# Coda-Research-Group/LearnedMetricIndex

Measured on AMD Instinct MI355X. Metric: queries/sec @ recall@10, 768-d 10M index, 10k query batch, higher is better.
Workload: dtype f16 prefilter (f32 accumulate) + f32 exact re-rank; outputs identical to the all-f32 path

## Files before the change

learnedmetricindex_amd/csrc/lmi_host_scan.h:

```cpp
#pragma once
#include "lmi_host.h"

static bool rescore_is_streamed(const lmi_index* h) {
    return h->rescore_streamed && rc_waves_for(h->dp, 4) > 0 && rc_wave_lds(h->dp, 4, true) <= RC_SMALL_LDS_CAP;
}
static int rescore_group_size(int nb) { return nb % 4 == 0 ? 4 : nb % 3 == 0 ? 3 : nb % 2 == 0 ? 2 : 1; }

struct ScanPlan {
    int nq, nb, kout, L;
    long long nslots;
    long long ncb_bound;
    long long ncols;
    int max_nch;
    long long part_lists;
    bool fast;
    bool low_d;
    bool ps_wide;
    int tile_cb;
    int sample_max;
    bool qbound;
    int primary_nb;
    bool use_front;
    bool streamed;
    int G, groups, sub_cap;
// ... 470 lines not shown
    F2.x.cap = 0;
    F2.x.fail = fbw + 2;
    F2.x.launch = 1;
    F2.head = F.head + 16;
    F2.redo_count = rc; F2.redo_bucket = rb; F2.redo_col = rcol;
    CHK(launch_pass2<false>(h, C.P, F2));
    return 0;
}

static void rescore_params(lmi_index* h, const ScanCall& C, const PrefilterParams& F, bool overflow_sorted, RescoreParams& Q) {
    const ScanPlan& P = C.P;
    unsigned* fbw = h->fb_list.as<unsigned>();
    Q.bucket_order = C.order;
    Q.slot_col = h->slot_col.as<int>();
    Q.nslots = (int)P.nslots;
    Q.nb = P.nb;
    Q.d = h->d;
    Q.raw = C.raw;
    Q.rb_start = h->d_rb_start.as<int>();
    Q.nb_rows = C.R.nb_rows;
    Q.cand_cnt = F.cand_cnt;
    Q.cand_row = F.cand_row;
    Q.cand_s = F.cand_s;
    Q.eps2 = F.eps2;
    Q.rows = h->rowmajor.as<float>();
    Q.dp = h->dp;
    Q.q = C.q;
    Q.qn2 = C.qn2;
    Q.ids_slab = h->ids_slab.as<unsigned>();
    Q.rank_d = h->rank_d.as<float>();
    Q.rank_id = h->rank_id.as<unsigned>();
    Q.fallback = h->fallback.as<int>();
    Q.nkeep = h->nkeep.as<int>();
    Q.fb_count = reinterpret_cast<int*>(fbw);
    Q.fb_list = reinterpret_cast<int*>(fbw + 8);
    Q.x_fail = fbw + 1;
    Q.x_off = overflow_sorted ? h->x_off.as<unsigned>() : nullptr;
    Q.x_ext = h->x_ext.as<uint2>();
    Q.x_log = F.x.log;
    Q.x_head = F.x.head;
    Q.x_cap = F.x.cap;
    Q.redo_col = overflow_sorted ? reinterpret_cast<const unsigned char*>(h->redo.as<unsigned>() + 1 + P.L) : nullptr;
    Q.ts = h->ts_set;
    Q.p2_end = p2_end_cell(h);
    if (Q.ts) { (void)tsp(h, ST_TAIL); (void)tsp(h, ST_P2END); (void)tsp(h, ST_FB); }
    Q.merge_pending = nullptr; Q.m_kout = 0; Q.m_out_d = nullptr; Q.m_out_id = nullptr; Q.m_out_key = nullptr;
#ifndef LMI_ABL_NOEMIT
    if (P.tail_merges) {
        Q.merge_pending = h->rs_flag.as<int>(); Q.m_kout = P.kout; Q.m_out_d = C.out_d; Q.m_out_id = C.out_id; Q.m_out_key = C.out_key;
        if (Q.ts) (void)tsp(h, ST_END);
    }
#endif
    Q.host_oflag = P.use_tail ? h->h_oflag : nullptr;
}
static Frag16 frag16_of(const lmi_index* h) {
    Frag16 F;
    F.frag = h->slab16.as<uint4>(); F.scale = h->xscale.as<float>(); F.KG16 = h->KG16; F.f16x16 = frag16x16(h);
    return F;
}

static int rerank(lmi_index* h, const ScanCall& C, const RescoreParams& Q) {
    const ScanPlan& P = C.P;
    const int nslots = (int)P.nslots, G = P.G, groups = P.groups;
    const bool f16 = h->storage == LMI_STORAGE_F16;
    if (!P.streamed) {
        if (f16) select_rescore_kernel<true><<<cdiv(nslots, RS_WAVES), 64 * RS_WAVES, 0, h->stream>>>(Q, frag16_of(h));
        else select_rescore_kernel<false><<<cdiv(nslots, RS_WAVES), 64 * RS_WAVES, 0, h->stream>>>(Q);
        HIPCHK(hipGetLastError());
        return 0;
    }
    CHK(h->surv_row.reserve((size_t)nslots * RC_KEEP * 4));
    SelectOut O;
    O.surv_row = h->surv_row.as<unsigned>();
    O.G = G;
    O.grp_flag = P.use_tail ? nullptr : h->rs_flag.as<int>();
    O.active = h->rs_active.as<int>();
    O.sub_cap = P.sub_cap;
    O.big = O.active + RC_SUB + RC_SUB * P.sub_cap;
    if (P.use_tail) {
        TailParams T;
        T.ngroups = groups; T.merge = P.tail_merges ? 1 : 0; T.kout = P.kout;
        T.out_d = C.out_d; T.out_id = C.out_id; T.out_key = C.out_key;
        T.pending = h->rs_flag.as<int>();
        const int lds_s = RC_WAVES * tail_wave_lds(h->dp, G, true);
        const int blocks = cdiv(groups, RC_WAVES);
#define LMI_TL_LAUNCH(GV) { if (f16) tail_kernel<GV, true><<<blocks, 64 * RC_WAVES, lds_s, h->stream>>>(Q, O, T, frag16_of(h)); \
                           else tail_kernel<GV><<<blocks, 64 * RC_WAVES, lds_s, h->stream>>>(Q, O, T); }
        if (G == 4) LMI_TL_LAUNCH(4) else if (G == 3) LMI_TL_LAUNCH(3) else if (G == 2) LMI_TL_LAUNCH(2) else LMI_TL_LAUNCH(1)
#undef LMI_TL_LAUNCH
        HIPCHK(hipGetLastError());
        return 0;
    }
    select_kernel<<<cdiv(nslots, 4), 256, 0, h->stream>>>(Q, O);
    HIPCHK(hipGetLastError());
    const int wb = rc_waves_for(h->dp, G), ws = rescore_small_waves(h->dp, G);
    h->last_plan[LMI_PLAN_RESCORE_SMALL_WAVES] = ws;
    const int blocks = cdiv(groups, ws);
    const int lds = wb * rc_wave_lds(h->dp, G), lds_s = ws * rc_wave_lds(h->dp, G, true);
#define LMI_RC_LAUNCH(GV) { if (f16) { rescore_kernel<GV, true, true><<<blocks, 64 * ws, lds_s, h->stream>>>(Q, O, frag16_of(h)); \
                                       rescore_kernel<GV, false, true><<<std::min(cdiv(groups, wb), h->num_cus), 64 * wb, lds, h->stream>>>(Q, O, frag16_of(h)); } \
                            else { rescore_kernel<GV, true><<<blocks, 64 * ws, lds_s, h->stream>>>(Q, O); \
                                   rescore_kernel<GV, false><<<std::min(cdiv(groups, wb), h->num_cus), 64 * wb, lds, h->stream>>>(Q, O); } }
    if (G == 4) LMI_RC_LAUNCH(4) else if (G == 3) LMI_RC_LAUNCH(3) else if (G == 2) LMI_RC_LAUNCH(2) else LMI_RC_LAUNCH(1)
#undef LMI_RC_LAUNCH
    HIPCHK(hipGetLastError());
    return 0;
}

static int scan_fallback(lmi_index* h, const ScanCall& C, const RescoreParams& Q) {
    if (h->storage == LMI_STORAGE_F16) fallback_kernel<true><<<std::min(cdiv(C.P.nslots, 4), h->num_cus * 4), 256, 0, h->stream>>>(Q, frag16_of(h));
    else fallback_kernel<false><<<std::min(cdiv(C.P.nslots, 4), h->num_cus * 4), 256, 0, h->stream>>>(Q);
    HIPCHK(hipGetLastError());
    return 0;
}

static int final_merge(lmi_index* h, const ScanCall& C) {
    const ScanPlan& P = C.P;
    const RouteArrays& R = C.R;
    MergeParams M;
    M.bucket_order = C.order;
    M.slot_col = h->slot_col.as<int>();
    M.nq = P.nq;
    M.nb = P.nb;
    M.L = P.L;
    M.kout = P.kout;
    M.raw = C.raw;
    M.skip_a = P.fast ? 1 : 0;
    M.rb_start = h->d_rb_start.as<int>();
    M.nb_rows = R.nb_rows;
    M.nch = R.nch;
    M.cb_start = R.cb_start;
    M.part_base = R.part_base;
    M.part_score = h->part_score.as<float>();
    M.part_row = h->part_row.as<unsigned>();
    M.ids_slab = h->ids_slab.as<unsigned>();
    M.qn2 = C.qn2;
    M.rank_d = h->rank_d.as<float>();
    M.rank_id = h->rank_id.as<unsigned>();
    M.ts = h->ts_set;
    M.scan_end = (!P.fast && h->ts_set) ? scan_end_cell(h) : nullptr;
    if (M.ts && !P.tail_merges) { (void)tsp(h, ST_MERGE); (void)tsp(h, ST_END); }
    M.out_d = C.out_d;
    M.out_id = C.out_id;
    M.out_key = C.out_key;
    const int kind = merge_kind(P);
    if (kind == 0) {  }
    else if (kind == 1) merge_ranks_kernel<<<cdiv(P.nq, 64), 64, 0, h->stream>>>(M);
    else merge_kernel<<<P.nq, 64, 0, h->stream>>>(M);
    HIPCHK(hipGetLastError());
    h->last_plan[LMI_PLAN_MERGE_KIND] = kind;
    return 0;
}

static int scan_enqueue(lmi_index* h, const float* d_qs, int nq, const int* d_order, int nb, int kout, int raw,
                        float* d_dists, uint32_t* d_ids, uint32_t* d_keys) {
    ScanCall C;
    C.P = scan_plan(h, nq, nb, kout);
    const ScanPlan& P = C.P;
    C.order = d_order; C.raw = raw;
    C.out_d = d_dists; C.out_id = d_ids; C.out_key = d_keys;
    plan_record(h, P, h->last_plan);
    CHK(scan_augment_l2(h, C, d_qs));
    CHK(scan_reserve(h, C));
    scan_route_arrays(h, P, C.R);
    CHK(P.use_front ? front_fused(h, C) : front_separate(h, C));
    if (!P.fast) {
        CHK(exact_scan(h, C));
    } else {
        CHK(record(h, 2));
        PrefilterParams F;
        prefilter_params(h, C, F);
        CHK(prefilter_passes(h, C, F));
        bool overflow_sorted = false;
        CHK(overflow_arm(h, P, &overflow_sorted));
        if (overflow_sorted) CHK(overflow_redo(h, C, F));
        h->last_plan[LMI_PLAN_OVERFLOW_SORTED] = overflow_sorted;
        RescoreParams Q;
        rescore_params(h, C, F, overflow_sorted, Q);
#ifndef LMI_ABL_NOEMIT
        CHK(rerank(h, C, Q));
#endif
// ... 42 lines not shown
```

learnedmetricindex_amd/csrc/lmi_rescore.h:

```cpp
#pragma once
#include <type_traits>

#include "lmi_prefilter.h"

namespace lmi {

#ifndef LMI_RC_ROWS
#define LMI_RC_ROWS 64
#endif
#ifndef LMI_RC_CHUNK
#define LMI_RC_CHUNK 32
#endif
#ifndef LMI_RC_DEPTH
#define LMI_RC_DEPTH 3
#endif
#ifndef LMI_RC_KEEP
#define LMI_RC_KEEP 256
#endif
constexpr int RC_ROWS = LMI_RC_ROWS;
constexpr int RC_CHUNK = LMI_RC_CHUNK;
constexpr int RC_DEPTH = LMI_RC_DEPTH;
constexpr int RC_KEEP = LMI_RC_KEEP;
constexpr int RC_PITCH = RC_CHUNK * 4 + 16;
constexpr int RC_PIECES = (RC_ROWS * RC_PITCH + 1023) / 1024;
// ... 39 lines not shown
                if (PERV <= 4 || i < nper) c += (int)__popcll(__ballot(key[i] >= probe));
            if (c >= KPB) T = probe;
        }
        pv = __uint_as_float(T ^ ((T >> 31) ? 0x80000000u : 0xffffffffu));
    }
    const float cut = pv - e2;
    const unsigned cbits = __float_as_uint(cut);
    const unsigned kcut = cut != cut ? 1u : cbits ^ ((cbits >> 31) ? 0xffffffffu : 0x80000000u);
    unsigned* out = O.surv_row + (size_t)p * RC_KEEP;
    unsigned nk = 0;
#pragma unroll
    for (int i = 0; i < PERV; ++i) {
        if (i < nper) {
            const bool keep = key[i] != 0u && key[i] >= kcut;
            const unsigned long long bal = __ballot(keep);
            if (keep) {
                const unsigned k = nk + (unsigned)__popcll(bal & ((1ull << lane) - 1ull));
                if (k < (unsigned)RC_KEEP) out[k] = row_base + (i < SPEC ? r_spec[i < SPEC ? i : 0] : cr[lane + 64 * i]);
            }
            nk += (unsigned)__popcll(bal);
        }
    }
    if (nk == 0u && lane < KPB) {
        const int b = bkt;
        const int rb0 = P.rb_start[b], n_b = P.nb_rows[b];
        P.rank_d[(size_t)p * KPB + lane] = P.raw ? -3.402823466e+38f : pad_dist(P.qn2);
        P.rank_id[(size_t)p * KPB + lane] = P.raw ? NOROW : P.ids_slab[(size_t)rb0 * 32 + (n_b - 1)];
    }
    if (lane == 0) {
        if (nk > (unsigned)RC_KEEP) flag_fallback(P, p);
        else {
            P.nkeep[p] = (int)nk;
            if (nk > 0 && atomicExch(&O.grp_flag[p / O.G], 1) == 0) {
                const int g = p / O.G, sub = g % RC_SUB;
                O.active[RC_SUB + sub * O.sub_cap + atomicAdd(&O.active[sub], 1)] = g;
            }
        }
    }
}

__global__ __launch_bounds__(256) void select_kernel(RescoreParams P, SelectOut O) {
    select_stamps(P);
    pf_x_scatter(P, blockIdx.x * 256 + threadIdx.x, gridDim.x * 256);
    const int wv = threadIdx.x >> 6, lane = threadIdx.x & 63;
    const int p = blockIdx.x * 4 + wv;
    if (p >= P.nslots) return;
    const float FMAXV = 3.402823466e+38f;
    const int col = P.slot_col[p];
    if (lane == 0) { P.fallback[p] = 0; P.nkeep[p] = 0; }
    if (col < 0) {
        if (lane < KPB) {
            P.rank_d[(size_t)p * KPB + lane] = P.raw ? -FMAXV : INFINITY;
            P.rank_id[(size_t)p * KPB + lane] = P.raw ? NOROW : 0u;
        }
        return;
    }
    const float* cs = P.cand_s + (size_t)col * PF_CAP;
    const unsigned* cr = P.cand_row + (size_t)col * PF_CAP;
    constexpr int PER = PF_CAP / 64;
    constexpr int SPEC = 4;
    float s_spec[SPEC];
    unsigned r_spec[SPEC];
#pragma unroll
    for (int i = 0; i < SPEC; ++i) { s_spec[i] = cs[lane + 64 * i]; r_spec[i] = cr[lane + 64 * i]; }
    const unsigned cnt = P.cand_cnt[col];
    if (cnt > (unsigned)PF_CAP) {
        if (lane == 0) flag_fallback(P, p);
        return;
    }
    if (cnt <= 64u) select_tail<1, SPEC>(P, O, p, col, lane, cnt, cs, cr, s_spec, r_spec);
    else if (cnt <= 256u) select_tail<4, SPEC>(P, O, p, col, lane, cnt, cs, cr, s_spec, r_spec);
    else select_tail<PER, SPEC>(P, O, p, col, lane, cnt, cs, cr, s_spec, r_spec);
}

constexpr int RC_SMALL_ROWS = 28;
#ifndef LMI_RC_SMALL_RING
#define LMI_RC_SMALL_RING (8 * 1024)
#endif
constexpr int RC_SMALL_LDS_CAP = 64 * 1024 + RC_WAVES * (LMI_RC_SMALL_RING - 8 * 1024);
constexpr int RC_SMALL_RING = LMI_RC_SMALL_RING;
__host__ __device__ inline int rc_wave_lds(int d, int G, bool small_form = false) {
    return small_form ? RC_SMALL_RING + d * 4 + 32 * 8 : RC_DEPTH * RC_BUF + d * 4 + G * RC_KEEP * 8;
}
__host__ inline int rc_waves_for(int d, int G) {
    for (int w = RC_WAVES; w >= 1; w >>= 1)
        if (w * rc_wave_lds(d, G) <= 160 * 1024 - 512) return w;
    return 0;
}
static_assert(RC_CHUNK % 32 == 0 && (RC_ROWS == 32 || RC_ROWS == 64) && RC_DEPTH >= 2 && RC_DEPTH <= 4, "rescore_kernel shapes");

template <int G, bool SMALL>
struct RcWave {
    static constexpr int RINGB = SMALL ? RC_SMALL_RING : RC_DEPTH * RC_BUF;
    static constexpr int KEEPW = SMALL ? 32 : G * RC_KEEP;
    unsigned char* mine;
    float* qs;
    unsigned* krow;
    float* ksc;
    __device__ __forceinline__ RcWave(unsigned char* base, int d) : mine(base), qs(reinterpret_cast<float*>(base + RINGB)),
        krow(reinterpret_cast<unsigned*>(base + RINGB + d * 4)), ksc(reinterpret_cast<float*>(base + RINGB + d * 4) + KEEPW) {}
    __device__ __forceinline__ void stage_query(const RescoreParams& P, int q, int lane) const {
        const int d = P.dp;
        const float* qg = P.q + (size_t)q * P.d;
        if (P.d == d) {
            for (int k = lane * 4; k < d; k += 256) *reinterpret_cast<float4*>(qs + k) = *reinterpret_cast<const float4*>(qg + k);
        } else {
            for (int k = lane; k < d; k += 64) qs[k] = k < P.d ? qg[k] : 0.0f;
        }
    }
};

template <int NP, int RINGB, bool H = false>
__device__ __forceinline__ void rc_run_batch(const RescoreParams& P, const Frag16& F, unsigned char* mine, const unsigned* krow, float* ksc, unsigned qaddr,
                                             int base, int total, int lane) {
    const int d = P.dp;
    const int n8 = (P.d + 7) >> 3;
    const int nchunks = H ? (n8 + 7) >> 3 : (d + RC_CHUNK - 1) / RC_CHUNK;
    float inv = 1.0f;
    if constexpr (H) inv = F.scale[1];
        constexpr int BUFB = NP * 1024;
        constexpr int DEPTH_RAW = RINGB / BUFB;
        constexpr int DEPTH = DEPTH_RAW > 16 ? 16 : ((DEPTH_RAW - 1) * NP > 60 ? 60 / NP + 1 : DEPTH_RAW);
        static_assert(DEPTH >= 2 && (DEPTH - 1) * NP <= 63, "vmcnt literal");
        const int nrows = min(RC_ROWS, total - base);
        const float* src[NP];
        unsigned colb[NP];
        int poff[H ? NP : 1];
#pragma unroll
        for (int pc = 0; pc < NP; ++pc) {
            const int o = pc * 1024 + lane * 16;
            const int r = o / RC_PITCH;
            const int cb = o - r * RC_PITCH;
            const bool okl = r < nrows && cb < RC_CHUNK * 4;
            const int i = base + (okl ? r : 0);
            if constexpr (H) {
                poff[pc] = okl ? 4 * frag16_piece_off(cb / 16, F.f16x16) : 0;
                src[pc] = reinterpret_cast<const float*>(F.frag + frag16_piece((long long)krow[i], 0, F.KG16, F.f16x16)) + poff[pc];
            } else {
                src[pc] = P.rows + (size_t)krow[i] * d + (okl ? cb / 4 : 0);
            }
            colb[pc] = okl ? (unsigned)cb : 0u;
        }
        auto issue = [&](int c, unsigned char* buf) {
            const int cbytes = H ? min(8, n8 - c * 8) * 16 : min(RC_CHUNK, d - c * RC_CHUNK) * 4;
#pragma unroll
            for (int pc = 0; pc < NP; ++pc) {
                const float* s_;
                if constexpr (H) s_ = src[pc] + c * 1024 - ((int)colb[pc] < cbytes ? 0 : poff[pc]);
                else s_ = src[pc] + c * RC_CHUNK - ((int)colb[pc] < cbytes ? 0 : (int)colb[pc] / 4);
                glds16(reinterpret_cast<const float4*>(s_), reinterpret_cast<float4*>(buf + pc * 1024));
            }
        };
        float acc = 0.0f;
#pragma unroll
        for (int c = 0; c < DEPTH - 1; ++c)
            if (c < nchunks) issue(c, mine + c * BUFB);
        int slot = 0;
        for (int c = 0; c < nchunks; ++c) {
            unsigned char* cur = mine + slot * BUFB;
            if (c + DEPTH - 1 < nchunks) {
                issue(c + DEPTH - 1, mine + (slot == 0 ? DEPTH - 1 : slot - 1) * BUFB);
                asm volatile("s_waitcnt vmcnt(%0)" :: "n"((DEPTH - 1) * NP) : "memory");
            } else {
                asm volatile("s_waitcnt vmcnt(0)" ::: "memory");
            }
            slot = slot + 1 == DEPTH ? 0 : slot + 1;
            if constexpr (H) {
              if (lane < nrows) {
                typedef float f32x4 __attribute__((ext_vector_type(4)));
                const unsigned xa = (unsigned)reinterpret_cast<uintptr_t>(cur) + (unsigned)lane * RC_PITCH;
                const unsigned qa = qaddr + (unsigned)c * 256u;
                const int np8 = min(8, n8 - c * 8);
                for (int st = 0; st * 4 < np8; ++st) {
                    f32x4 xv[4], qq[8];
                    const unsigned xo = xa + st * 64u, qo = qa + st * 128u;
                    asm volatile("ds_read_b128 %0, %12\n\tds_read_b128 %1, %12 offset:16\n\tds_read_b128 %2, %12 offset:32\n\t"
                                 "ds_read_b128 %3, %12 offset:48\n\t"
                                 "ds_read_b128 %4, %13\n\tds_read_b128 %5, %13 offset:16\n\tds_read_b128 %6, %13 offset:32\n\t"
                                 "ds_read_b128 %7, %13 offset:48\n\tds_read_b128 %8, %13 offset:64\n\tds_read_b128 %9, %13 offset:80\n\t"
                                 "ds_read_b128 %10, %13 offset:96\n\tds_read_b128 %11, %13 offset:112\n\ts_waitcnt lgkmcnt(0)"
                                 : "=&v"(xv[0]), "=&v"(xv[1]), "=&v"(xv[2]), "=&v"(xv[3]),
                                   "=&v"(qq[0]), "=&v"(qq[1]), "=&v"(qq[2]), "=&v"(qq[3]), "=&v"(qq[4]), "=&v"(qq[5]), "=&v"(qq[6]), "=&v"(qq[7])
                                 : "v"(xo), "v"(qo) : "memory");
                    const int nv = min(4, np8 - st * 4);
#pragma unroll
                    for (int t = 0; t < 4; ++t) {
                        if (t < nv) {
                            const half8 hv = __builtin_bit_cast(half8, xv[t]);
                            acc = __builtin_fmaf(qq[2 * t].x, (float)hv[0] * inv, acc); acc = __builtin_fmaf(qq[2 * t].y, (float)hv[1] * inv, acc);
                            acc = __builtin_fmaf(qq[2 * t].z, (float)hv[2] * inv, acc); acc = __builtin_fmaf(qq[2 * t].w, (float)hv[3] * inv, acc);
                            acc = __builtin_fmaf(qq[2 * t + 1].x, (float)hv[4] * inv, acc); acc = __builtin_fmaf(qq[2 * t + 1].y, (float)hv[5] * inv, acc);
                            acc = __builtin_fmaf(qq[2 * t + 1].z, (float)hv[6] * inv, acc); acc = __builtin_fmaf(qq[2 * t + 1].w, (float)hv[7] * inv, acc);
                        }
                    }
                }
              }
            } else if (lane < nrows) {
                typedef float f32x4 __attribute__((ext_vector_type(4)));
                const unsigned xa = (unsigned)reinterpret_cast<uintptr_t>(cur) + (unsigned)lane * RC_PITCH;
                const unsigned qa = qaddr + (unsigned)c * RC_CHUNK * 4u;
                const int nsteps = (min(RC_CHUNK, d - c * RC_CHUNK) + 31) / 32;
                const int tail = min(RC_CHUNK, d - c * RC_CHUNK) - (nsteps - 1) * 32;
                for (int st = 0; st < nsteps; ++st) {
                    f32x4 xv[8], qq[8];
                    const unsigned xo = xa + st * 128u, qo = qa + st * 128u;
                    asm volatile("ds_read_b128 %0, %16\n\tds_read_b128 %1, %16 offset:16\n\tds_read_b128 %2, %16 offset:32\n\t"
                                 "ds_read_b128 %3, %16 offset:48\n\tds_read_b128 %4, %16 offset:64\n\tds_read_b128 %5, %16 offset:80\n\t"
                                 "ds_read_b128 %6, %16 offset:96\n\tds_read_b128 %7, %16 offset:112\n\t"
                                 "ds_read_b128 %8, %17\n\tds_read_b128 %9, %17 offset:16\n\tds_read_b128 %10, %17 offset:32\n\t"
                                 "ds_read_b128 %11, %17 offset:48\n\tds_read_b128 %12, %17 offset:64\n\tds_read_b128 %13, %17 offset:80\n\t"
                                 "ds_read_b128 %14, %17 offset:96\n\tds_read_b128 %15, %17 offset:112\n\ts_waitcnt lgkmcnt(0)"
                                 : "=&v"(xv[0]), "=&v"(xv[1]), "=&v"(xv[2]), "=&v"(xv[3]), "=&v"(xv[4]), "=&v"(xv[5]), "=&v"(xv[6]), "=&v"(xv[7]),
                                   "=&v"(qq[0]), "=&v"(qq[1]), "=&v"(qq[2]), "=&v"(qq[3]), "=&v"(qq[4]), "=&v"(qq[5]), "=&v"(qq[6]), "=&v"(qq[7])
                                 : "v"(xo), "v"(qo) : "memory");
                    const int nv = st + 1 < nsteps ? 8 : tail / 4;
#pragma unroll
                    for (int t = 0; t < 8; ++t) {
                        if (t < nv) {
                            acc = __builtin_fmaf(qq[t].x, xv[t].x, acc); acc = __builtin_fmaf(qq[t].y, xv[t].y, acc);
                            acc = __builtin_fmaf(qq[t].z, xv[t].z, acc); acc = __builtin_fmaf(qq[t].w, xv[t].w, acc);
                        }
                    }
                }
            }
        }
        if (lane < nrows) ksc[base + lane] = acc;
}
template <bool SMALL, bool H = false>
__device__ __forceinline__ void rc_stream_batch(const RescoreParams& P, const Frag16& F, unsigned char* mine, const unsigned* krow, float* ksc, unsigned qaddr,
                                                int base, int total, int lane) {
    constexpr int RINGB = SMALL ? RC_SMALL_RING : RC_DEPTH * RC_BUF;
    const int np = (min(RC_ROWS, total - base) * RC_PITCH + 1023) / 1024;
    if (np <= 2) rc_run_batch<2, RINGB, H>(P, F, mine, krow, ksc, qaddr, base, total, lane);
    else if (SMALL || (np <= 4 && RC_PIECES > 4)) rc_run_batch<(RC_PIECES > 4 ? 4 : RC_PIECES), RINGB, H>(P, F, mine, krow, ksc, qaddr, base, total, lane);
    else { if constexpr (!SMALL) rc_run_batch<RC_PIECES, RINGB, H>(P, F, mine, krow, ksc, qaddr, base, total, lane); }
}

template <int G, bool SMALL, bool LCOPY, bool PRE = false, bool H = false>
__device__ __forceinline__ void rescore_core(const RescoreParams& P, const Frag16& F, const RcWave<G, SMALL>& W, const int (&off)[G + 1], int p0, int lane,
                                             const int (&colv)[G], const int (&fbv)[G], float* rl_d, unsigned* rl_i,
                                             unsigned my_id = 0u, const unsigned* row_base = nullptr, const int* nbr = nullptr, const unsigned* pad_id = nullptr) {
    unsigned char* mine = W.mine;
    unsigned* krow = W.krow;
    float* ksc = W.ksc;
    const float FMAXV = 3.402823466e+38f;
    const int total = off[G];
    const unsigned qaddr = (unsigned)reinterpret_cast<uintptr_t>(W.qs);
    for (int base = 0; base < total; base += RC_ROWS) rc_stream_batch<SMALL, H>(P, F, mine, krow, ksc, qaddr, base, total, lane);
    __builtin_amdgcn_fence(__ATOMIC_ACQ_REL, "wavefront");
    __builtin_amdgcn_wave_barrier();
    for (int base = 0; base < total; base += 64) {
        const int i = base + lane;
        if (i < total) {
            int sl = 0;
#pragma unroll
            for (int t = 1; t < G; ++t) sl += i >= off[t] ? 1 : 0;
            int lo = off[0], hi = off[1];
#pragma unroll
            for (int t = 1; t < G; ++t) { lo = sl == t ? off[t] : lo; hi = sl == t ? off[t + 1] : hi; }
            const float sc = ksc[i];
            const unsigned row = krow[i];
            int pos = 0;
            for (int j = lo; j < hi; ++j) pos += better(ksc[j], krow[j], sc, row) ? 1 : 0;
            if (pos < KPB) {
                const int p = p0 + sl;
                const float dv = P.raw ? sc : sim_to_dist(sc, P.qn2, p / P.nb);
                unsigned iv;
                if constexpr (PRE) {
                    unsigned rbase = row_base[0];
#pragma unroll
                    for (int t = 1; t < G; ++t) rbase = sl == t ? row_base[t] : rbase;
                    iv = P.raw ? row - rbase : my_id;
                } else {
                    iv = P.raw ? row - (unsigned)P.rb_start[P.bucket_order[p]] * 32u : P.ids_slab[row];
                }
                P.rank_d[(size_t)p * KPB + pos] = dv;
                P.rank_id[(size_t)p * KPB + pos] = iv;
                if (LCOPY) { rl_d[sl * KPB + pos] = dv; rl_i[sl * KPB + pos] = iv; }
            }
        }
    }
    if (lane < KPB) {
#pragma unroll
        for (int sl = 0; sl < G; ++sl) {
            const int p = p0 + sl;
            if (colv[sl] < 0 || fbv[sl]) continue;
            int n_b;
            unsigned pad_iv;
            if constexpr (PRE) {
                n_b = nbr[sl];
                pad_iv = pad_id[sl];
            } else {
                const int b = P.bucket_order[p];
                const int rb0 = P.rb_start[b];
                n_b = P.nb_rows[b];
                pad_iv = P.raw ? NOROW : P.ids_slab[(size_t)rb0 * 32 + (n_b - 1)];
            }
            const int nreal = min(min(off[sl + 1] - off[sl], KPB), n_b);
            if (lane >= nreal) {
                const float dv = P.raw ? -FMAXV : pad_dist(P.qn2);
                const unsigned iv = P.raw ? NOROW : pad_iv;
                P.rank_d[(size_t)p * KPB + lane] = dv;
                P.rank_id[(size_t)p * KPB + lane] = iv;
                if (LCOPY) { rl_d[sl * KPB + lane] = dv; rl_i[sl * KPB + lane] = iv; }
            }
        }
    }
}

template <int G, bool SMALL, bool H = false>
__device__ __forceinline__ void rescore_group(const RescoreParams& P, const Frag16& F, const SelectOut& O, unsigned char* rc_smem, int wv, int lane, int p0) {
    const int d = P.dp;
    const RcWave<G, SMALL> W(rc_smem + (size_t)wv * rc_wave_lds(d, G, SMALL), d);
    int off[G + 1];
    off[0] = 0;
    int colv[G], fbv[G], nkv[G];
#pragma unroll
    for (int sl = 0; sl < G; ++sl) { colv[sl] = P.slot_col[p0 + sl]; fbv[sl] = P.fallback[p0 + sl]; nkv[sl] = P.nkeep[p0 + sl]; }
#pragma unroll
    for (int sl = 0; sl < G; ++sl) off[sl + 1] = off[sl] + ((colv[sl] >= 0 && !fbv[sl]) ? nkv[sl] : 0);
    if (SMALL && off[G] > RC_SMALL_ROWS) {
        if (lane == 0) O.big[1 + atomicAdd(&O.big[0], 1)] = p0 / G;
        return;
    }
#pragma unroll
    for (int sl = 0; sl < G; ++sl) {
        const int nk = off[sl + 1] - off[sl];
        for (int i = lane; i < nk; i += 64) W.krow[off[sl] + i] = O.surv_row[(size_t)(p0 + sl) * RC_KEEP + i];
    }
    W.stage_query(P, p0 / P.nb, lane);
    __builtin_amdgcn_fence(__ATOMIC_ACQ_REL, "wavefront");
    __builtin_amdgcn_wave_barrier();
    rescore_core<G, SMALL, false, false, H>(P, F, W, off, p0, lane, colv, fbv, nullptr, nullptr);
}

template <int G, bool SMALL, bool H = false, class... FR>
__global__ __launch_bounds__(64 * RC_WAVES, SMALL ? 3 : 1) void rescore_kernel(RescoreParams P, SelectOut O, FR... frag) {
    extern __shared__ __attribute__((aligned(16))) unsigned char rc_smem[];
    const Frag16 F = frag16_arg(frag...);
    const int wv = __builtin_amdgcn_readfirstlane(threadIdx.x >> 6), lane = threadIdx.x & 63;
    const int nwv = (int)(blockDim.x >> 6);
    const int wid = blockIdx.x * nwv + wv;
    if (SMALL) {
        int incl = O.active[lane];
#pragma unroll
        for (int o = 1; o < 64; o <<= 1) {
            const int up = __shfl_up(incl, o, 64);
            if (lane >= o) incl += up;
        }
        const int sub = (int)__popcll(__ballot(incl <= wid));
        if (sub >= RC_SUB) return;
        const int before = sub ? __shfl(incl, sub - 1, 64) : 0;
        rescore_group<G, true, H>(P, F, O, rc_smem, wv, lane, O.active[RC_SUB + sub * O.sub_cap + (wid - before)] * G);
    } else {
        const int nbig = __builtin_amdgcn_readfirstlane(O.big[0]);
        for (int i = wid; i < nbig; i += (int)gridDim.x * nwv) {
            rescore_group<G, false, H>(P, F, O, rc_smem, wv, lane, O.big[1 + i] * G);
            __builtin_amdgcn_fence(__ATOMIC_ACQ_REL, "wavefront");
            __builtin_amdgcn_wave_barrier();
        }
    }
}

}
```

learnedmetricindex_amd/csrc/lmi_tail.h:

```cpp
#pragma once
#include "lmi_rescore.h"

namespace lmi {

struct TailParams {
    int ngroups;
    int merge;
    int kout;
    float* out_d;
    unsigned* out_id;
    unsigned* out_key;
    int* pending;
};

__host__ __device__ inline int tail_wave_lds(int d, int G, bool small_form) { return (rc_wave_lds(d, G, small_form) + 15) / 16 * 16 + 4 * G * KPB * 4; }

template <int PERV, int SPEC>
__device__ __forceinline__ unsigned tail_select(int lane, unsigned cnt, float e2, unsigned row_base, const float* __restrict__ cs,
                                                const unsigned* __restrict__ cr, const float (&s_spec)[SPEC], const unsigned (&r_spec)[SPEC],
                                                unsigned* __restrict__ out_g, unsigned* krow_l, int cap_l) {
    const int nper = (int)((cnt + 63u) >> 6);
    unsigned key[PERV];
#pragma unroll
    for (int i = 0; i < PERV; ++i) {
        const int e = lane + 64 * i;
        key[i] = 0u;
        if (i < nper && e < (int)cnt) {
            const unsigned bits = __float_as_uint(i < SPEC ? s_spec[i < SPEC ? i : 0] : cs[e]);
            key[i] = bits ^ ((bits >> 31) ? 0xffffffffu : 0x80000000u);
        }
    }
    float pv = -INFINITY;
    if (cnt >= (unsigned)KPB) {
        unsigned T = 0;
        for (int bit = 31; bit >= 0; --bit) {
            const unsigned probe = T | (1u << bit);
            int c = 0;
#pragma unroll
            for (int i = 0; i < PERV; ++i)
                if (PERV <= 4 || i < nper) c += (int)__popcll(__ballot(key[i] >= probe));
            if (c >= KPB) T = probe;
        }
        pv = __uint_as_float(T ^ ((T >> 31) ? 0x80000000u : 0xffffffffu));
    }
    const float cut = pv - e2;
    const unsigned cbits = __float_as_uint(cut);
    const unsigned kcut = cut != cut ? 1u : cbits ^ ((cbits >> 31) ? 0xffffffffu : 0x80000000u);
    unsigned nk = 0;
#pragma unroll
    for (int i = 0; i < PERV; ++i) {
        if (i < nper) {
            const bool keep = key[i] != 0u && key[i] >= kcut;
            const unsigned long long bal = __ballot(keep);
            if (keep) {
                const unsigned k = nk + (unsigned)__popcll(bal & ((1ull << lane) - 1ull));
                const unsigned row = row_base + (i < SPEC ? r_spec[i < SPEC ? i : 0] : cr[lane + 64 * i]);
                if (k < (unsigned)RC_KEEP) out_g[k] = row;
                if ((int)k < cap_l) krow_l[k] = row;
            }
            nk += (unsigned)__popcll(bal);
        }
    }
    return nk;
}

template <int G, bool H = false, class... FR>
__global__ __launch_bounds__(64 * RC_WAVES, 3) void tail_kernel(RescoreParams P, SelectOut O, TailParams T, FR... frag) {
    select_stamps(P);
    pf_x_scatter(P, blockIdx.x * blockDim.x + threadIdx.x, gridDim.x * blockDim.x);
    extern __shared__ __attribute__((aligned(16))) unsigned char tl_smem[];
    const Frag16 F = frag16_arg(frag...);
    const int wv = __builtin_amdgcn_readfirstlane(threadIdx.x >> 6), lane = threadIdx.x & 63;
    const int nwv = (int)(blockDim.x >> 6);
    const int grp = blockIdx.x * nwv + wv;
    if (grp >= T.ngroups) return;
    const int q = (grp * G) / P.nb;
    const int dp = P.dp;
    unsigned char* base = tl_smem + (size_t)wv * tail_wave_lds(dp, G, true);
    const RcWave<G, true> W(base, dp);
    float* rl_d = reinterpret_cast<float*>(base + (rc_wave_lds(dp, G, true) + 15) / 16 * 16);
    unsigned* rl_i = reinterpret_cast<unsigned*>(rl_d + G * KPB);
    const int p0 = grp * G;
    const float FMAXV = 3.402823466e+38f;
    constexpr int SPEC = 4;
    constexpr int PER = PF_CAP / 64;
    int colv[G], fbv[G], off[G + 1], bkt[G], nbr[G];
    unsigned cnt[G], row_base[G], pad_id[G];
    float e2[G];
    float s_spec[G][SPEC];
    unsigned r_spec[G][SPEC];
#pragma unroll
    for (int sl = 0; sl < G; ++sl) { colv[sl] = P.slot_col[p0 + sl]; bkt[sl] = P.bucket_order[p0 + sl]; }
    W.stage_query(P, q, lane);
#pragma unroll
    for (int sl = 0; sl < G; ++sl) {
        const size_t c = (size_t)(colv[sl] < 0 ? 0 : colv[sl]);
        if (colv[sl] < 0) bkt[sl] = 0;
        cnt[sl] = colv[sl] < 0 ? 0u : P.cand_cnt[c];
        e2[sl] = colv[sl] < 0 ? 0.0f : P.eps2[c];
        row_base[sl] = colv[sl] < 0 ? 0u : (unsigned)P.rb_start[bkt[sl]] * 32u;
        nbr[sl] = colv[sl] < 0 ? 0 : P.nb_rows[bkt[sl]];
#pragma unroll
        for (int i = 0; i < SPEC; ++i) {
            s_spec[sl][i] = colv[sl] < 0 ? 0.0f : P.cand_s[c * PF_CAP + lane + 64 * i];
            r_spec[sl][i] = colv[sl] < 0 ? 0u : P.cand_row[c * PF_CAP + lane + 64 * i];
        }
    }
#pragma unroll
    for (int sl = 0; sl < G; ++sl) pad_id[sl] = (colv[sl] < 0 || P.raw || nbr[sl] <= 0) ? NOROW : P.ids_slab[(size_t)row_base[sl] + (unsigned)(nbr[sl] - 1)];
    off[0] = 0;
    int nflag = 0;
#pragma unroll
    for (int sl = 0; sl < G; ++sl) {
        const int p = p0 + sl;
        off[sl + 1] = off[sl];
        fbv[sl] = 0;
        int nkeep = 0;
        if (colv[sl] < 0) {
            if (lane < KPB) {
                const float dv = P.raw ? -FMAXV : INFINITY;
                const unsigned iv = P.raw ? NOROW : 0u;
                P.rank_d[(size_t)p * KPB + lane] = dv;
                P.rank_id[(size_t)p * KPB + lane] = iv;
                rl_d[sl * KPB + lane] = dv;
                rl_i[sl * KPB + lane] = iv;
            }
        } else if (cnt[sl] > (unsigned)PF_CAP) {
            fbv[sl] = 1;
        } else {
            const float* cs = P.cand_s + (size_t)colv[sl] * PF_CAP;
            const unsigned* cr = P.cand_row + (size_t)colv[sl] * PF_CAP;
            unsigned* out_g = O.surv_row + (size_t)p * RC_KEEP;
            unsigned* krow_l = W.krow + off[sl];
            const int cap_l = RcWave<G, true>::KEEPW - off[sl];
            unsigned nk;
            if (cnt[sl] <= 64u) nk = tail_select<1, SPEC>(lane, cnt[sl], e2[sl], row_base[sl], cs, cr, s_spec[sl], r_spec[sl], out_g, krow_l, cap_l);
            else if (cnt[sl] <= 256u) nk = tail_select<4, SPEC>(lane, cnt[sl], e2[sl], row_base[sl], cs, cr, s_spec[sl], r_spec[sl], out_g, krow_l, cap_l);
            else nk = tail_select<PER, SPEC>(lane, cnt[sl], e2[sl], row_base[sl], cs, cr, s_spec[sl], r_spec[sl], out_g, krow_l, cap_l);
            if (nk > (unsigned)RC_KEEP) fbv[sl] = 1;
            else { nkeep = (int)nk; off[sl + 1] = off[sl] + (int)nk; }
        }
        if (lane == 0) {
            P.nkeep[p] = nkeep;
            if (fbv[sl]) flag_fallback(P, p); else P.fallback[p] = 0;
        }
        nflag += fbv[sl];
    }
    if (lane == 0 && T.merge) T.pending[q] = nflag;
    const int total = off[G];
    __builtin_amdgcn_fence(__ATOMIC_ACQ_REL, "wavefront");
    __builtin_amdgcn_wave_barrier();
    if (total <= RC_SMALL_ROWS) {
        const unsigned my_id = (lane < total && !P.raw) ? P.ids_slab[W.krow[lane]] : 0u;
        rescore_core<G, true, true, true, H>(P, F, W, off, p0, lane, colv, fbv, rl_d, rl_i, my_id, row_base, nbr, pad_id);
    } else {
        float* best_s = reinterpret_cast<float*>(rl_i + G * KPB);
        unsigned* best_r = reinterpret_cast<unsigned*>(best_s + G * KPB);
        int nbest[G];
#pragma unroll
        for (int sl = 0; sl < G; ++sl) nbest[sl] = 0;
        const unsigned qaddr = (unsigned)reinterpret_cast<uintptr_t>(W.qs);
        asm volatile("s_waitcnt vmcnt(0)" ::: "memory");
        for (int base = 0; base < total; base += RC_SMALL_ROWS) {
            const int nrows = min(RC_SMALL_ROWS, total - base);
            if (lane < nrows) {
                const int e = base + lane;
                int sl = 0;
#pragma unroll
                for (int t = 1; t < G; ++t) sl += e >= off[t] ? 1 : 0;
                int lo = off[0];
#pragma unroll
                for (int t = 1; t < G; ++t) lo = sl == t ? off[t] : lo;
                W.krow[lane] = __builtin_nontemporal_load(O.surv_row + (size_t)(p0 + sl) * RC_KEEP + (e - lo));
            }
            __builtin_amdgcn_fence(__ATOMIC_ACQ_REL, "wavefront");
            __builtin_amdgcn_wave_barrier();
            rc_stream_batch<true, H>(P, F, W.mine, W.krow, W.ksc, qaddr, 0, nrows, lane);
            __builtin_amdgcn_fence(__ATOMIC_ACQ_REL, "wavefront");
            __builtin_amdgcn_wave_barrier();
#pragma unroll
            for (int sl = 0; sl < G; ++sl) {
                const int b_lo = max(off[sl], base) - base, b_hi = min(off[sl + 1], base + nrows) - base;
                const int nbat = max(0, b_hi - b_lo), nold = nbest[sl], n = nold + nbat;
                if (nbat > 0) {
                    float sc = -INFINITY;
                    unsigned row = NOROW;
                    if (lane < nold) { sc = best_s[sl * KPB + lane]; row = best_r[sl * KPB + lane]; }
                    else if (lane < n) { sc = W.ksc[b_lo + lane - nold]; row = W.krow[b_lo + lane - nold]; }
                    int pos = 0;
                    for (int o = 0; o < n; ++o) {
                        const float os = __builtin_bit_cast(float, __builtin_amdgcn_readlane(__builtin_bit_cast(int, sc), o));
                        const unsigned orr = (unsigned)__builtin_amdgcn_readlane((int)row, o);
                        pos += better(os, orr, sc, row) ? 1 : 0;
                    }
                    if (lane < n && pos < KPB) { best_s[sl * KPB + pos] = sc; best_r[sl * KPB + pos] = row; }
                    nbest[sl] = min(n, KPB);
                }
            }
            __builtin_amdgcn_fence(__ATOMIC_ACQ_REL, "wavefront");
            __builtin_amdgcn_wave_barrier();
        }
        if (lane < KPB) {
#pragma unroll
            for (int sl = 0; sl < G; ++sl) {
                const int p = p0 + sl;
                if (colv[sl] < 0 || fbv[sl]) continue;
                const int b = P.bucket_order[p];
                const int rb0 = P.rb_start[b], n_b = P.nb_rows[b];
                const int nreal = min(nbest[sl], n_b);
                float dv;
                unsigned iv;
                if (lane < nreal) {
                    const float sc = best_s[sl * KPB + lane];
                    const unsigned row = best_r[sl * KPB + lane];
                    dv = P.raw ? sc : sim_to_dist(sc, P.qn2, q);
                    iv = P.raw ? row - (unsigned)rb0 * 32u : P.ids_slab[row];
                } else {
                    dv = P.raw ? -FMAXV : pad_dist(P.qn2);
                    iv = P.raw ? NOROW : P.ids_slab[(size_t)rb0 * 32 + (n_b - 1)];
                }
                P.rank_d[(size_t)p * KPB + lane] = dv;
                P.rank_id[(size_t)p * KPB + lane] = iv;
                rl_d[sl * KPB + lane] = dv;
                rl_i[sl * KPB + lane] = iv;
            }
        }
    }
    if (nflag || !T.merge) return;
    __builtin_amdgcn_fence(__ATOMIC_ACQ_REL, "wavefront");
    __builtin_amdgcn_wave_barrier();
    const float dv = lane < G * KPB ? rl_d[lane] : 0.0f;
    const unsigned iv = lane < G * KPB ? rl_i[lane] : 0u;
    merge_entries<G>(dv, iv, lane, P.raw, T.kout, (size_t)q, T.out_d, T.out_id, T.out_key);
}

}
```

Measured before the change: 2.088 million.

## Read query vector via scalar loads instead of staging it in LDS

Removes the per-wave LDS copy of the query vector in the rescore and tail kernels. The query is now read through a wave-uniform constant-address-space pointer, so scalar loads of 32 floats are broadcast per step, with a lane-held register tail for the ragged end, a lookahead prefetch and an early cache-touch of the row. Dropping d*4 bytes of LDS per wave shrinks the launch LDS size, and the launch bounds for the small and tail kernels rise from 3 to 4 blocks. In exchange, the inner loop depends on scalar memory latency and more registers (32 floats of qq), which could raise register pressure.

Measured after the change: 2.096 million, median of 6. About the same (+0.4%).

```diff
diff --git a/learnedmetricindex_amd/csrc/lmi_host_scan.h b/learnedmetricindex_amd/csrc/lmi_host_scan.h
--- a/learnedmetricindex_amd/csrc/lmi_host_scan.h
+++ b/learnedmetricindex_amd/csrc/lmi_host_scan.h
@@ -576,7 +576,7 @@
         T.ngroups = groups; T.merge = P.tail_merges ? 1 : 0; T.kout = P.kout;
         T.out_d = C.out_d; T.out_id = C.out_id; T.out_key = C.out_key;
         T.pending = h->rs_flag.as<int>();
-        const int lds_s = RC_WAVES * tail_wave_lds(h->dp, G, true);
+        const int lds_s = RC_WAVES * tail_wave_lds_launch(G, true);
         const int blocks = cdiv(groups, RC_WAVES);
 #define LMI_TL_LAUNCH(GV) { if (f16) tail_kernel<GV, true><<<blocks, 64 * RC_WAVES, lds_s, h->stream>>>(Q, O, T, frag16_of(h)); \
                            else tail_kernel<GV><<<blocks, 64 * RC_WAVES, lds_s, h->stream>>>(Q, O, T); }
@@ -590,7 +590,7 @@
     const int wb = rc_waves_for(h->dp, G), ws = rescore_small_waves(h->dp, G);
     h->last_plan[LMI_PLAN_RESCORE_SMALL_WAVES] = ws;
     const int blocks = cdiv(groups, ws);
-    const int lds = wb * rc_wave_lds(h->dp, G), lds_s = ws * rc_wave_lds(h->dp, G, true);
+    const int lds = wb * rc_wave_lds_launch(G), lds_s = ws * rc_wave_lds_launch(G, true);
 #define LMI_RC_LAUNCH(GV) { if (f16) { rescore_kernel<GV, true, true><<<blocks, 64 * ws, lds_s, h->stream>>>(Q, O, frag16_of(h)); \
                                        rescore_kernel<GV, false, true><<<std::min(cdiv(groups, wb), h->num_cus), 64 * wb, lds, h->stream>>>(Q, O, frag16_of(h)); } \
                             else { rescore_kernel<GV, true><<<blocks, 64 * ws, lds_s, h->stream>>>(Q, O); \
diff --git a/learnedmetricindex_amd/csrc/lmi_rescore.h b/learnedmetricindex_amd/csrc/lmi_rescore.h
--- a/learnedmetricindex_amd/csrc/lmi_rescore.h
+++ b/learnedmetricindex_amd/csrc/lmi_rescore.h
@@ -145,6 +145,9 @@
 __host__ __device__ inline int rc_wave_lds(int d, int G, bool small_form = false) {
     return small_form ? RC_SMALL_RING + d * 4 + 32 * 8 : RC_DEPTH * RC_BUF + d * 4 + G * RC_KEEP * 8;
 }
+__host__ __device__ inline int rc_wave_lds_launch(int G, bool small_form = false) {
+    return small_form ? RC_SMALL_RING + 32 * 8 : RC_DEPTH * RC_BUF + G * RC_KEEP * 8;
+}
 __host__ inline int rc_waves_for(int d, int G) {
     for (int w = RC_WAVES; w >= 1; w >>= 1)
         if (w * rc_wave_lds(d, G) <= 160 * 1024 - 512) return w;
@@ -157,24 +160,48 @@
     static constexpr int RINGB = SMALL ? RC_SMALL_RING : RC_DEPTH * RC_BUF;
     static constexpr int KEEPW = SMALL ? 32 : G * RC_KEEP;
     unsigned char* mine;
-    float* qs;
     unsigned* krow;
     float* ksc;
-    __device__ __forceinline__ RcWave(unsigned char* base, int d) : mine(base), qs(reinterpret_cast<float*>(base + RINGB)),
-        krow(reinterpret_cast<unsigned*>(base + RINGB + d * 4)), ksc(reinterpret_cast<float*>(base + RINGB + d * 4) + KEEPW) {}
-    __device__ __forceinline__ void stage_query(const RescoreParams& P, int q, int lane) const {
-        const int d = P.dp;
-        const float* qg = P.q + (size_t)q * P.d;
-        if (P.d == d) {
-            for (int k = lane * 4; k < d; k += 256) *reinterpret_cast<float4*>(qs + k) = *reinterpret_cast<const float4*>(qg + k);
-        } else {
-            for (int k = lane; k < d; k += 64) qs[k] = k < P.d ? qg[k] : 0.0f;
-        }
-    }
+    __device__ __forceinline__ explicit RcWave(unsigned char* base) : mine(base),
+        krow(reinterpret_cast<unsigned*>(base + RINGB)), ksc(reinterpret_cast<float*>(base + RINGB) + KEEPW) {}
 };
 
+typedef const __attribute__((address_space(4))) float* RcQRow;
+__device__ __forceinline__ RcQRow rc_query_row(const RescoreParams& P, int q) {
+    const unsigned long long a = reinterpret_cast<unsigned long long>(P.q + (size_t)q * P.d);
+    const unsigned lo = (unsigned)__builtin_amdgcn_readfirstlane((int)(unsigned)a), hi = (unsigned)__builtin_amdgcn_readfirstlane((int)(unsigned)(a >> 32));
+    return reinterpret_cast<RcQRow>(((unsigned long long)hi << 32) | lo);
+}
+__device__ __forceinline__ float rc_q_tail(RcQRow qrow, int klast, int d, int lane) {
+    const float* qg = reinterpret_cast<const float*>(reinterpret_cast<unsigned long long>(qrow));
+    const int k = klast + lane;
+    return (klast + 32 > d && lane < 32 && k < d) ? qg[k] : 0.0f;
+}
+__device__ __forceinline__ void rc_q_step(RcQRow qrow, int k0, int d, float qtail, float (&qv)[32]) {
+    if (k0 + 32 <= d) {
+#pragma unroll
+        for (int t = 0; t < 32; ++t) qv[t] = qrow[k0 + t];
+    } else {
+        asm volatile("" : "+v"(qtail));
+#pragma unroll
+        for (int t = 0; t < 32; ++t) qv[t] = __builtin_bit_cast(float, __builtin_amdgcn_readlane(__builtin_bit_cast(int, qtail), t));
+    }
+}
+
+struct RcQAhead { float a = 0.0f, b = 0.0f; };
+__device__ __forceinline__ void rc_q_ahead_retire(const RcQAhead& A) { asm volatile("" :: "s"(A.a), "s"(A.b)); }
+__device__ __forceinline__ void rc_q_ahead(RcQRow qrow, int k0, int d, RcQAhead& A) {
+    rc_q_ahead_retire(A);
+    A.a = qrow[min(k0, d - 1)];
+    A.b = qrow[min(k0 + 16, d - 1)];
+}
+__device__ __forceinline__ float rc_touch_query(const RescoreParams& P, int q, int lane) {
+    return (P.q + (size_t)q * P.d)[min(lane * 16, P.d - 1)];
+}
+__device__ __forceinline__ void rc_touch_retire(float t) { asm volatile("" :: "v"(t)); }
+
 template <int NP, int RINGB, bool H = false>
-__device__ __forceinline__ void rc_run_batch(const RescoreParams& P, const Frag16& F, unsigned char* mine, const unsigned* krow, float* ksc, unsigned qaddr,
+__device__ __forceinline__ void rc_run_batch(const RescoreParams& P, const Frag16& F, unsigned char* mine, const unsigned* krow, float* ksc, RcQRow qrow,
                                              int base, int total, int lane) {
     const int d = P.dp;
     const int n8 = (P.d + 7) >> 3;
@@ -215,12 +242,17 @@
             }
         };
         float acc = 0.0f;
+        const float qtail = rc_q_tail(qrow, (((H ? n8 * 8 : d) - 1) >> 5) << 5, P.d, lane);
 #pragma unroll
         for (int c = 0; c < DEPTH - 1; ++c)
             if (c < nchunks) issue(c, mine + c * BUFB);
+        int kq = 0;
+        RcQAhead ahead;
         int slot = 0;
         for (int c = 0; c < nchunks; ++c) {
             unsigned char* cur = mine + slot * BUFB;
+            float qq[32];
+            rc_q_step(qrow, kq, P.d, qtail, qq);
             if (c + DEPTH - 1 < nchunks) {
                 issue(c + DEPTH - 1, mine + (slot == 0 ? DEPTH - 1 : slot - 1) * BUFB);
                 asm volatile("s_waitcnt vmcnt(%0)" :: "n"((DEPTH - 1) * NP) : "memory");
@@ -228,75 +260,69 @@
                 asm volatile("s_waitcnt vmcnt(0)" ::: "memory");
             }
             slot = slot + 1 == DEPTH ? 0 : slot + 1;
+            typedef float f32x4 __attribute__((ext_vector_type(4)));
+            const unsigned xa = (unsigned)reinterpret_cast<uintptr_t>(cur) + (unsigned)min(lane, nrows - 1) * RC_PITCH;
             if constexpr (H) {
-              if (lane < nrows) {
-                typedef float f32x4 __attribute__((ext_vector_type(4)));
-                const unsigned xa = (unsigned)reinterpret_cast<uintptr_t>(cur) + (unsigned)lane * RC_PITCH;
-                const unsigned qa = qaddr + (unsigned)c * 256u;
                 const int np8 = min(8, n8 - c * 8);
                 for (int st = 0; st * 4 < np8; ++st) {
-                    f32x4 xv[4], qq[8];
-                    const unsigned xo = xa + st * 64u, qo = qa + st * 128u;
-                    asm volatile("ds_read_b128 %0, %12\n\tds_read_b128 %1, %12 offset:16\n\tds_read_b128 %2, %12 offset:32\n\t"
-                                 "ds_read_b128 %3, %12 offset:48\n\t"
-                                 "ds_read_b128 %4, %13\n\tds_read_b128 %5, %13 offset:16\n\tds_read_b128 %6, %13 offset:32\n\t"
-                                 "ds_read_b128 %7, %13 offset:48\n\tds_read_b128 %8, %13 offset:64\n\tds_read_b128 %9, %13 offset:80\n\t"
-                                 "ds_read_b128 %10, %13 offset:96\n\tds_read_b128 %11, %13 offset:112\n\ts_waitcnt lgkmcnt(0)"
-                                 : "=&v"(xv[0]), "=&v"(xv[1]), "=&v"(xv[2]), "=&v"(xv[3]),
-                                   "=&v"(qq[0]), "=&v"(qq[1]), "=&v"(qq[2]), "=&v"(qq[3]), "=&v"(qq[4]), "=&v"(qq[5]), "=&v"(qq[6]), "=&v"(qq[7])
-                                 : "v"(xo), "v"(qo) : "memory");
-                    const int nv = min(4, np8 - st * 4);
-#pragma unroll
-                    for (int t = 0; t < 4; ++t) {
-                        if (t < nv) {
-                            const half8 hv = __builtin_bit_cast(half8, xv[t]);
-                            acc = __builtin_fmaf(qq[2 * t].x, (float)hv[0] * inv, acc); acc = __builtin_fmaf(qq[2 * t].y, (float)hv[1] * inv, acc);
-                            acc = __builtin_fmaf(qq[2 * t].z, (float)hv[2] * inv, acc); acc = __builtin_fmaf(qq[2 * t].w, (float)hv[3] * inv, acc);
-                            acc = __builtin_fmaf(qq[2 * t + 1].x, (float)hv[4] * inv, acc); acc = __builtin_fmaf(qq[2 * t + 1].y, (float)hv[5] * inv, acc);
-                            acc = __builtin_fmaf(qq[2 * t + 1].z, (float)hv[6] * inv, acc); acc = __builtin_fmaf(qq[2 * t + 1].w, (float)hv[7] * inv, acc);
+                    if (st > 0) rc_q_step(qrow, kq, P.d, qtail, qq);
+                    kq += 32;
+                    {
+                        f32x4 xv[4];
+                        const unsigned xo = xa + st * 64u;
+                        asm volatile("ds_read_b128 %0, %4\n\tds_read_b128 %1, %4 offset:16\n\tds_read_b128 %2, %4 offset:32\n\t"
+                                     "ds_read_b128 %3, %4 offset:48\n\ts_waitcnt lgkmcnt(0)"
+                                     : "=&v"(xv[0]), "=&v"(xv[1]), "=&v"(xv[2]), "=&v"(xv[3]) : "v"(xo) : "memory");
+                        rc_q_ahead(qrow, kq, P.d, ahead);
+                        const int nv = min(4, np8 - st * 4);
+#pragma unroll
+                        for (int t = 0; t < 4; ++t) {
+                            if (t < nv) {
+                                const half8 hv = __builtin_bit_cast(half8, xv[t]);
+#pragma unroll
+                                for (int j = 0; j < 8; ++j) acc = __builtin_fmaf(qq[8 * t + j], (float)hv[j] * inv, acc);
+                            }
                         }
                     }
                 }
-              }
-            } else if (lane < nrows) {
-                typedef float f32x4 __attribute__((ext_vector_type(4)));
-                const unsigned xa = (unsigned)reinterpret_cast<uintptr_t>(cur) + (unsigned)lane * RC_PITCH;
-                const unsigned qa = qaddr + (unsigned)c * RC_CHUNK * 4u;
+            } else {
                 const int nsteps = (min(RC_CHUNK, d - c * RC_CHUNK) + 31) / 32;
                 const int tail = min(RC_CHUNK, d - c * RC_CHUNK) - (nsteps - 1) * 32;
                 for (int st = 0; st < nsteps; ++st) {
-                    f32x4 xv[8], qq[8];
-                    const unsigned xo = xa + st * 128u, qo = qa + st * 128u;
-                    asm volatile("ds_read_b128 %0, %16\n\tds_read_b128 %1, %16 offset:16\n\tds_read_b128 %2, %16 offset:32\n\t"
-                                 "ds_read_b128 %3, %16 offset:48\n\tds_read_b128 %4, %16 offset:64\n\tds_read_b128 %5, %16 offset:80\n\t"
-                                 "ds_read_b128 %6, %16 offset:96\n\tds_read_b128 %7, %16 offset:112\n\t"
-                                 "ds_read_b128 %8, %17\n\tds_read_b128 %9, %17 offset:16\n\tds_read_b128 %10, %17 offset:32\n\t"
-                                 "ds_read_b128 %11, %17 offset:48\n\tds_read_b128 %12, %17 offset:64\n\tds_read_b128 %13, %17 offset:80\n\t"
-                                 "ds_read_b128 %14, %17 offset:96\n\tds_read_b128 %15, %17 offset:112\n\ts_waitcnt lgkmcnt(0)"
-                                 : "=&v"(xv[0]), "=&v"(xv[1]), "=&v"(xv[2]), "=&v"(xv[3]), "=&v"(xv[4]), "=&v"(xv[5]), "=&v"(xv[6]), "=&v"(xv[7]),
-                                   "=&v"(qq[0]), "=&v"(qq[1]), "=&v"(qq[2]), "=&v"(qq[3]), "=&v"(qq[4]), "=&v"(qq[5]), "=&v"(qq[6]), "=&v"(qq[7])
-                                 : "v"(xo), "v"(qo) : "memory");
-                    const int nv = st + 1 < nsteps ? 8 : tail / 4;
-#pragma unroll
-                    for (int t = 0; t < 8; ++t) {
-                        if (t < nv) {
-                            acc = __builtin_fmaf(qq[t].x, xv[t].x, acc); acc = __builtin_fmaf(qq[t].y, xv[t].y, acc);
-                            acc = __builtin_fmaf(qq[t].z, xv[t].z, acc); acc = __builtin_fmaf(qq[t].w, xv[t].w, acc);
+                    if (st > 0) rc_q_step(qrow, kq, P.d, qtail, qq);
+                    kq += 32;
+                    {
+                        f32x4 xv[8];
+                        const unsigned xo = xa + st * 128u;
+                        asm volatile("ds_read_b128 %0, %8\n\tds_read_b128 %1, %8 offset:16\n\tds_read_b128 %2, %8 offset:32\n\t"
+                                     "ds_read_b128 %3, %8 offset:48\n\tds_read_b128 %4, %8 offset:64\n\tds_read_b128 %5, %8 offset:80\n\t"
+                                     "ds_read_b128 %6, %8 offset:96\n\tds_read_b128 %7, %8 offset:112\n\ts_waitcnt lgkmcnt(0)"
+                                     : "=&v"(xv[0]), "=&v"(xv[1]), "=&v"(xv[2]), "=&v"(xv[3]), "=&v"(xv[4]), "=&v"(xv[5]), "=&v"(xv[6]), "=&v"(xv[7])
+                                     : "v"(xo) : "memory");
+                        rc_q_ahead(qrow, kq, P.d, ahead);
+                        const int nv = st + 1 < nsteps ? 8 : tail / 4;
+#pragma unroll
+                        for (int t = 0; t < 8; ++t) {
+                            if (t < nv) {
+                                acc = __builtin_fmaf(qq[4 * t], xv[t].x, acc); acc = __builtin_fmaf(qq[4 * t + 1], xv[t].y, acc);
+                                acc = __builtin_fmaf(qq[4 * t + 2], xv[t].z, acc); acc = __builtin_fmaf(qq[4 * t + 3], xv[t].w, acc);
+                            }
                         }
                     }
                 }
             }
         }
+        rc_q_ahead_retire(ahead);
         if (lane < nrows) ksc[base + lane] = acc;
 }
 template <bool SMALL, bool H = false>
-__device__ __forceinline__ void rc_stream_batch(const RescoreParams& P, const Frag16& F, unsigned char* mine, const unsigned* krow, float* ksc, unsigned qaddr,
+__device__ __forceinline__ void rc_stream_batch(const RescoreParams& P, const Frag16& F, unsigned char* mine, const unsigned* krow, float* ksc, RcQRow qrow,
                                                 int base, int total, int lane) {
     constexpr int RINGB = SMALL ? RC_SMALL_RING : RC_DEPTH * RC_BUF;
     const int np = (min(RC_ROWS, total - base) * RC_PITCH + 1023) / 1024;
-    if (np <= 2) rc_run_batch<2, RINGB, H>(P, F, mine, krow, ksc, qaddr, base, total, lane);
-    else if (SMALL || (np <= 4 && RC_PIECES > 4)) rc_run_batch<(RC_PIECES > 4 ? 4 : RC_PIECES), RINGB, H>(P, F, mine, krow, ksc, qaddr, base, total, lane);
-    else { if constexpr (!SMALL) rc_run_batch<RC_PIECES, RINGB, H>(P, F, mine, krow, ksc, qaddr, base, total, lane); }
+    if (np <= 2) rc_run_batch<2, RINGB, H>(P, F, mine, krow, ksc, qrow, base, total, lane);
+    else if (SMALL || (np <= 4 && RC_PIECES > 4)) rc_run_batch<(RC_PIECES > 4 ? 4 : RC_PIECES), RINGB, H>(P, F, mine, krow, ksc, qrow, base, total, lane);
+    else { if constexpr (!SMALL) rc_run_batch<RC_PIECES, RINGB, H>(P, F, mine, krow, ksc, qrow, base, total, lane); }
 }
 
 template <int G, bool SMALL, bool LCOPY, bool PRE = false, bool H = false>
@@ -308,8 +334,8 @@
     float* ksc = W.ksc;
     const float FMAXV = 3.402823466e+38f;
     const int total = off[G];
-    const unsigned qaddr = (unsigned)reinterpret_cast<uintptr_t>(W.qs);
-    for (int base = 0; base < total; base += RC_ROWS) rc_stream_batch<SMALL, H>(P, F, mine, krow, ksc, qaddr, base, total, lane);
+    const RcQRow qrow = rc_query_row(P, p0 / P.nb);
+    for (int base = 0; base < total; base += RC_ROWS) rc_stream_batch<SMALL, H>(P, F, mine, krow, ksc, qrow, base, total, lane);
     __builtin_amdgcn_fence(__ATOMIC_ACQ_REL, "wavefront");
     __builtin_amdgcn_wave_barrier();
     for (int base = 0; base < total; base += 64) {
@@ -373,8 +399,7 @@
 
 template <int G, bool SMALL, bool H = false>
 __device__ __forceinline__ void rescore_group(const RescoreParams& P, const Frag16& F, const SelectOut& O, unsigned char* rc_smem, int wv, int lane, int p0) {
-    const int d = P.dp;
-    const RcWave<G, SMALL> W(rc_smem + (size_t)wv * rc_wave_lds(d, G, SMALL), d);
+    const RcWave<G, SMALL> W(rc_smem + (size_t)wv * rc_wave_lds_launch(G, SMALL));
     int off[G + 1];
     off[0] = 0;
     int colv[G], fbv[G], nkv[G];
@@ -391,14 +416,15 @@
         const int nk = off[sl + 1] - off[sl];
         for (int i = lane; i < nk; i += 64) W.krow[off[sl] + i] = O.surv_row[(size_t)(p0 + sl) * RC_KEEP + i];
     }
-    W.stage_query(P, p0 / P.nb, lane);
+    const float qt = rc_touch_query(P, p0 / P.nb, lane);
     __builtin_amdgcn_fence(__ATOMIC_ACQ_REL, "wavefront");
     __builtin_amdgcn_wave_barrier();
     rescore_core<G, SMALL, false, false, H>(P, F, W, off, p0, lane, colv, fbv, nullptr, nullptr);
+    rc_touch_retire(qt);
 }
 
 template <int G, bool SMALL, bool H = false, class... FR>
-__global__ __launch_bounds__(64 * RC_WAVES, SMALL ? 3 : 1) void rescore_kernel(RescoreParams P, SelectOut O, FR... frag) {
+__global__ __launch_bounds__(64 * RC_WAVES, SMALL ? 4 : 1) void rescore_kernel(RescoreParams P, SelectOut O, FR... frag) {
     extern __shared__ __attribute__((aligned(16))) unsigned char rc_smem[];
     const Frag16 F = frag16_arg(frag...);
     const int wv = __builtin_amdgcn_readfirstlane(threadIdx.x >> 6), lane = threadIdx.x & 63;
diff --git a/learnedmetricindex_amd/csrc/lmi_tail.h b/learnedmetricindex_amd/csrc/lmi_tail.h
--- a/learnedmetricindex_amd/csrc/lmi_tail.h
+++ b/learnedmetricindex_amd/csrc/lmi_tail.h
@@ -14,6 +14,7 @@
 };
 
 __host__ __device__ inline int tail_wave_lds(int d, int G, bool small_form) { return (rc_wave_lds(d, G, small_form) + 15) / 16 * 16 + 4 * G * KPB * 4; }
+__host__ __device__ inline int tail_wave_lds_launch(int G, bool small_form) { return (rc_wave_lds_launch(G, small_form) + 15) / 16 * 16 + 4 * G * KPB * 4; }
 
 template <int PERV, int SPEC>
 __device__ __forceinline__ unsigned tail_select(int lane, unsigned cnt, float e2, unsigned row_base, const float* __restrict__ cs,
@@ -65,7 +66,7 @@
 }
 
 template <int G, bool H = false, class... FR>
-__global__ __launch_bounds__(64 * RC_WAVES, 3) void tail_kernel(RescoreParams P, SelectOut O, TailParams T, FR... frag) {
+__global__ __launch_bounds__(64 * RC_WAVES, 4) void tail_kernel(RescoreParams P, SelectOut O, TailParams T, FR... frag) {
     select_stamps(P);
     pf_x_scatter(P, blockIdx.x * blockDim.x + threadIdx.x, gridDim.x * blockDim.x);
     extern __shared__ __attribute__((aligned(16))) unsigned char tl_smem[];
@@ -75,10 +76,9 @@
     const int grp = blockIdx.x * nwv + wv;
     if (grp >= T.ngroups) return;
     const int q = (grp * G) / P.nb;
-    const int dp = P.dp;
-    unsigned char* base = tl_smem + (size_t)wv * tail_wave_lds(dp, G, true);
-    const RcWave<G, true> W(base, dp);
-    float* rl_d = reinterpret_cast<float*>(base + (rc_wave_lds(dp, G, true) + 15) / 16 * 16);
+    unsigned char* base = tl_smem + (size_t)wv * tail_wave_lds_launch(G, true);
+    const RcWave<G, true> W(base);
+    float* rl_d = reinterpret_cast<float*>(base + (rc_wave_lds_launch(G, true) + 15) / 16 * 16);
     unsigned* rl_i = reinterpret_cast<unsigned*>(rl_d + G * KPB);
     const int p0 = grp * G;
     const float FMAXV = 3.402823466e+38f;
@@ -91,7 +91,7 @@
     unsigned r_spec[G][SPEC];
 #pragma unroll
     for (int sl = 0; sl < G; ++sl) { colv[sl] = P.slot_col[p0 + sl]; bkt[sl] = P.bucket_order[p0 + sl]; }
-    W.stage_query(P, q, lane);
+    const float qt = rc_touch_query(P, q, lane);
 #pragma unroll
     for (int sl = 0; sl < G; ++sl) {
         const size_t c = (size_t)(colv[sl] < 0 ? 0 : colv[sl]);
@@ -148,6 +148,7 @@
     }
     if (lane == 0 && T.merge) T.pending[q] = nflag;
     const int total = off[G];
+    rc_touch_retire(qt);
     __builtin_amdgcn_fence(__ATOMIC_ACQ_REL, "wavefront");
     __builtin_amdgcn_wave_barrier();
     if (total <= RC_SMALL_ROWS) {
@@ -159,7 +160,7 @@
         int nbest[G];
 #pragma unroll
         for (int sl = 0; sl < G; ++sl) nbest[sl] = 0;
-        const unsigned qaddr = (unsigned)reinterpret_cast<uintptr_t>(W.qs);
+        const RcQRow qrow = rc_query_row(P, q);
         asm volatile("s_waitcnt vmcnt(0)" ::: "memory");
         for (int base = 0; base < total; base += RC_SMALL_ROWS) {
             const int nrows = min(RC_SMALL_ROWS, total - base);
@@ -175,7 +176,7 @@
             }
             __builtin_amdgcn_fence(__ATOMIC_ACQ_REL, "wavefront");
             __builtin_amdgcn_wave_barrier();
-            rc_stream_batch<true, H>(P, F, W.mine, W.krow, W.ksc, qaddr, 0, nrows, lane);
+            rc_stream_batch<true, H>(P, F, W.mine, W.krow, W.ksc, qrow, 0, nrows, lane);
             __builtin_amdgcn_fence(__ATOMIC_ACQ_REL, "wavefront");
             __builtin_amdgcn_wave_barrier();
 #pragma unroll
```
